# kongwanbianjinyu/PromptIR

Measured on AMD Instinct MI355X. Metric: 128x128 patches/sec (fwd+bwd train step, whole job), higher is better.
Workload: dtype f32 (bf16x3 split-MFMA, f32 accumulate)

## Files before the change

include/promptir_hip.h:

```cpp
#ifndef PROMPTIR_HIP_H
#define PROMPTIR_HIP_H

#include <stddef.h>
#include <stdint.h>

#ifdef __cplusplus
extern "C" {
#endif

#define PIR_OK 0
#define PIR_EINVAL (-22)
#define PIR_ENOMEM (-12)

typedef void* pir_stream_t;

int pir_abi_version(void);
const char* pir_arch(void);

int pir_tune_set(int knob, int value);

int pir_build_flags(void);

typedef struct {
  const float* A; long a_s1, a_s2; long a_sm, a_sk;
  const float* X; long x_s1, x_s2; long ldx;
  float* Y; long y_s1, y_s2; long ldy;
  const float* R; long r_s1, r_s2; long ldr;
  const float* rowscale; long rs_s1, rs_s2;
  int M, K, N;
  int O1, O2;
  const void* A3; int a3_kp;
} pir_gemm_nn_t;
int pir_gemm_nn(const pir_gemm_nn_t* args, pir_stream_t stream);
size_t pir_gemm_nn_ws_floats(const pir_gemm_nn_t* args);
int pir_gemm_nn_ws(const pir_gemm_nn_t* args, float* ws, size_t ws_floats, pir_stream_t stream);
int pir_ln_conv1x1_fwd(const float* x, long x_bs, const float* ln_w, const float* ln_b, const void* A3, int a3_kp,
                       float* y, long y_bs, float* mean_out, float* rstd_out, int B, int M, int K, int HW, pir_stream_t stream);
int pir_conv1x1_wgrad_ln(const float* dy, long dy_bs, const float* x, long x_bs, const float* mean, const float* rstd,
                         const float* ln_w, const float* ln_b, float* dw, float* ws, size_t ws_floats,
                         int B, int Cout, int Cin, int HW, pir_stream_t stream);

int pir_conv1x1_dgrad_ln_bwd(const float* dy, long dy_bs, const void* A3, int a3_kp, int K,
                             const float* x, long x_bs, const float* ln_w, const float* mean, const float* rstd,
                             const float* dres, long dres_bs, float* dx, long dx_bs, float* dweight, float* dbias,
                             float* ws, size_t ws_floats, int B, int C, int HW, pir_stream_t stream);

int pir_gemm_nn_plan(const pir_gemm_nn_t* args);
size_t pir_split_bf16x3_bytes(int M, int K);
int pir_split_bf16x3(const float* W, int M, int K, long sm, long sk, void* out, pir_stream_t stream);

int pir_conv3x3(const float* A, long a_st, long a_sm, long a_sk, int flip,
                const float* X, long x_bs, float* Y, long y_bs,
                const float* R, long r_bs,
                int B, int M, int K, int H, int W, pir_stream_t stream);

typedef struct {
  const float* X; long x_s1, x_s2, x_sr; long ldx;
  const float* Y; long y_s1, y_s2, y_sr; long ldy;
  float* G; long g_so, g_si, g_sj;
  int M1, M2, N;
  int O1, O2, BR;
  int shift_dh, shift_dw, H, W;
  float* ws; size_t ws_floats;
  float alpha;
  int accumulate;
} pir_gemm_nt_t;
size_t pir_gemm_nt_ws_floats(int M1, int M2, int N, int O, int BR);
int pir_gemm_nt(const pir_gemm_nt_t* args, pir_stream_t stream);
int pir_gemm_nt_partials(const pir_gemm_nt_t* args, int* splits, pir_stream_t stream);
int pir_gemm_nt_group(const pir_gemm_nt_t* probs, int n, pir_stream_t stream);
size_t pir_gemm_nt_ws_needed(const pir_gemm_nt_t* args);
size_t pir_gemm_nt_group_ws_needed(const pir_gemm_nt_t* probs, int n, int k);

int pir_split_bf16x3_taps(const float* W, int M, int K, long st, long sm, long sk, int flip, void* out,
                          pir_stream_t stream);
int pir_conv3x3_x3(const void* A3, int a3_kp, const float* X, long x_bs, float* Y, long y_bs,
                   const float* R, long r_bs, int B, int M, int K, int H, int W, pir_stream_t stream);
size_t pir_conv3x3_x3_ws_floats(int B, int M, int K, int H, int W);
int pir_conv3x3_x3_ws(const void* A3, int a3_kp, const float* X, long x_bs, float* Y, long y_bs,
                      const float* R, long r_bs, int B, int M, int K, int H, int W,
                      float* ws, size_t ws_floats, pir_stream_t stream);

typedef struct {
  const float* W; void* out;
  long st, sm, sk;
  int M, K, taps, flip;
} pir_split_desc_t;
int pir_split_bf16x3_batch(const pir_split_desc_t* descs, const int* blocks, int nblocks, pir_stream_t stream);

size_t pir_conv3x3_wgrad_ws_floats(int Cout, int Cin, int H, int W, int B);
int pir_conv3x3_wgrad(const float* dy, long dy_bs, const float* x, long x_bs, float* dw, int B, int Cout, int Cin,
                      int H, int W, float* ws, size_t ws_floats, int accumulate, pir_stream_t stream);

int pir_layernorm_fwd(const float* x, long x_bs, const float* weight, const float* bias,
                      float* y, long y_bs, float* mean, float* rstd,
                      int B, int C, int HW, pir_stream_t stream);
size_t pir_layernorm_bwd_ws_floats(int B, int C, int HW);
int pir_layernorm_bwd(const float* dy, long dy_bs, const float* x, long x_bs, const float* weight,
                      int with_bias, const float* mean, const float* rstd,
                      float* dx, long dx_bs, const float* dres, long dres_bs, float* dweight, float* dbias,
                      float* ws, size_t ws_floats, int B, int C, int HW, pir_stream_t stream);

int pir_dwconv3x3(const float* x, long x_bs, const float* w, int flip, float* y, long y_bs,
                  int B, int C, int H, int W, pir_stream_t stream);
size_t pir_dwconv3x3_sumsq_floats(int B, int nsq, int H);
int pir_dwconv3x3_sumsq(const float* x, long x_bs, const float* w, float* y, long y_bs, float* sq_parts,
                        size_t sq_floats, int nsq, int* nparts, int B, int C, int H, int W, pir_stream_t stream);
int pir_dwconv3x3_gate(const float* x, long x_bs, const float* w, float* g, long g_bs,
                       int B, int hid, int H, int W, pir_stream_t stream);
int pir_dwconv3x3_gate_bwd(const float* x, long x_bs, const float* w, const float* dg, long dg_bs,
                           float* dt, long dt_bs, int B, int hid, int H, int W, pir_stream_t stream);
size_t pir_dwconv3x3_wgrad_ws_floats(int B, int C, int H, int W);
int pir_dwconv3x3_wgrad(const float* dy, long dy_bs, const float* x, long x_bs, float* dw,
                        float* ws, size_t ws_floats, int B, int C, int H, int W, pir_stream_t stream);

size_t pir_dwconv3x3_bwd_ws_floats(int B, int C, int H, int W);
int pir_dwconv3x3_bwd(const float* dy, long dy_bs, const float* x, long x_bs, const float* w,
                      float* dx, long dx_bs, float* dw, float* ws, size_t ws_floats,
                      int B, int C, int H, int W, pir_stream_t stream);
size_t pir_gdfn_dwconv_bwd_ws_floats(int B, int hid, int H, int W);
int pir_gdfn_dwconv_bwd(const float* x, long x_bs, const float* w, const float* dg, long dg_bs,
                        float* dx, long dx_bs, float* dw, float* ws, size_t ws_floats,
                        int B, int hid, int H, int W, pir_stream_t stream);

int pir_row_sumsq(const float* x, long x_bs, float* out, int B, int C, int HW, pir_stream_t stream);
int pir_mdta_softmax_fwd(const float* gram, const float* sumsq, int nparts, const float* temperature,
                         float* attn, int B, int heads, int c, pir_stream_t stream);
int pir_mdta_softmax_fwd_parts(const float* gram_parts, int splits, const float* sumsq, int nparts,
                               const float* temperature, float* gram, float* attn, int B, int heads, int c,
                               pir_stream_t stream);
// ... 77 lines not shown
```

promptir_amd/_lib.py:

```python
from __future__ import annotations

import ctypes as C
import os

_HERE = os.path.dirname(os.path.abspath(__file__))
LIB_PATH = os.environ.get("PIR_LIB", os.path.join(_HERE, "libpromptir_hip.so"))
ABI_VERSION = 8

c_float_p = C.c_void_p
c_long = C.c_long
c_int = C.c_int
c_size_t = C.c_size_t
c_float = C.c_float
stream_t = C.c_void_p


class GemmNN(C.Structure):
    _fields_ = [
        ("A", c_float_p), ("a_s1", c_long), ("a_s2", c_long), ("a_sm", c_long), ("a_sk", c_long),
        ("X", c_float_p), ("x_s1", c_long), ("x_s2", c_long), ("ldx", c_long),
        ("Y", c_float_p), ("y_s1", c_long), ("y_s2", c_long), ("ldy", c_long),
        ("R", c_float_p), ("r_s1", c_long), ("r_s2", c_long), ("ldr", c_long),
        ("rowscale", c_float_p), ("rs_s1", c_long), ("rs_s2", c_long),
        ("M", c_int), ("K", c_int), ("N", c_int), ("O1", c_int), ("O2", c_int),
        ("A3", c_float_p), ("a3_kp", c_int),
    ]


class GemmNT(C.Structure):
    _fields_ = [
        ("X", c_float_p), ("x_s1", c_long), ("x_s2", c_long), ("x_sr", c_long), ("ldx", c_long),
        ("Y", c_float_p), ("y_s1", c_long), ("y_s2", c_long), ("y_sr", c_long), ("ldy", c_long),
        ("G", c_float_p), ("g_so", c_long), ("g_si", c_long), ("g_sj", c_long),
        ("M1", c_int), ("M2", c_int), ("N", c_int), ("O1", c_int), ("O2", c_int), ("BR", c_int),
        ("shift_dh", c_int), ("shift_dw", c_int), ("H", c_int), ("W", c_int),
        ("ws", c_float_p), ("ws_floats", c_size_t),
        ("alpha", c_float), ("accumulate", c_int),
    ]


class SplitDesc(C.Structure):
    _fields_ = [("W", c_float_p), ("out", c_float_p), ("st", c_long), ("sm", c_long), ("sk", c_long),
                ("M", c_int), ("K", c_int), ("taps", c_int), ("flip", c_int)]


P, L, I, Z, F, S = c_float_p, c_long, c_int, c_size_t, c_float, stream_t

SIGNATURES = {
    "pir_abi_version": (I, []),
    "pir_arch": (C.c_char_p, []),
    "pir_tune_set": (I, [I, I]),
    "pir_build_flags": (I, []),
    "pir_gemm_nn": (I, [C.POINTER(GemmNN), S]),
    "pir_gemm_nn_ws": (I, [C.POINTER(GemmNN), P, Z, S]),
    "pir_gemm_nn_ws_floats": (Z, [C.POINTER(GemmNN)]),
    "pir_gemm_nn_plan": (I, [C.POINTER(GemmNN)]),
    "pir_split_bf16x3_bytes": (Z, [I, I]),
    "pir_split_bf16x3": (I, [P, I, I, L, L, P, S]),
    "pir_conv3x3": (I, [P, L, L, L, I, P, L, P, L, P, L, I, I, I, I, I, S]),
    "pir_gemm_nt_ws_floats": (Z, [I, I, I, I, I]),
    "pir_gemm_nt": (I, [C.POINTER(GemmNT), S]),
    "pir_gemm_nt_partials": (I, [C.POINTER(GemmNT), C.POINTER(C.c_int), S]),
    "pir_gemm_nt_group": (I, [C.POINTER(GemmNT), I, S]),
    "pir_gemm_nt_ws_needed": (Z, [C.POINTER(GemmNT)]),
    "pir_gemm_nt_group_ws_needed": (Z, [C.POINTER(GemmNT), I, I]),
    "pir_split_bf16x3_batch": (I, [P, P, I, S]),
    "pir_split_bf16x3_taps": (I, [P, I, I, L, L, L, I, P, S]),
    "pir_conv3x3_x3": (I, [P, I, P, L, P, L, P, L, I, I, I, I, I, S]),
    "pir_conv3x3_x3_ws": (I, [P, I, P, L, P, L, P, L, I, I, I, I, I, P, Z, S]),
    "pir_conv3x3_x3_ws_floats": (Z, [I, I, I, I, I]),
    "pir_conv3x3_wgrad_ws_floats": (Z, [I, I, I, I, I]),
    "pir_conv3x3_wgrad": (I, [P, L, P, L, P, I, I, I, I, I, P, Z, I, S]),
    "pir_layernorm_fwd": (I, [P, L, P, P, P, L, P, P, I, I, I, S]),
    "pir_layernorm_bwd_ws_floats": (Z, [I, I, I]),
    "pir_layernorm_bwd": (I, [P, L, P, L, P, I, P, P, P, L, P, L, P, P, P, Z, I, I, I, S]),
    "pir_dwconv3x3": (I, [P, L, P, I, P, L, I, I, I, I, S]),
    "pir_dwconv3x3_gate": (I, [P, L, P, P, L, I, I, I, I, S]),
    "pir_dwconv3x3_gate_bwd": (I, [P, L, P, P, L, P, L, I, I, I, I, S]),
    "pir_dwconv3x3_wgrad_ws_floats": (Z, [I, I, I, I]),
    "pir_dwconv3x3_wgrad": (I, [P, L, P, L, P, P, Z, I, I, I, I, S]),
    "pir_dwconv3x3_bwd_ws_floats": (Z, [I, I, I, I]),
    "pir_dwconv3x3_bwd": (I, [P, L, P, L, P, P, L, P, P, Z, I, I, I, I, S]),
    "pir_gdfn_dwconv_bwd_ws_floats": (Z, [I, I, I, I]),
    "pir_gdfn_dwconv_bwd": (I, [P, L, P, P, L, P, L, P, P, Z, I, I, I, I, S]),
    "pir_gdfn_fused_ws_bytes": (Z, [I, I, I, I]),
    "pir_gdfn_fused_fwd": (I, [P, L, P, P, P, I, P, P, L, P, Z, P, P, I, I, I, I, I, S]),
    "pir_row_sumsq": (I, [P, L, P, I, I, I, S]),
    "pir_mdta_softmax_fwd": (I, [P, P, I, P, P, I, I, I, S]),
    "pir_mdta_softmax_bwd": (I, [P, P, P, P, I, P, P, P, P, P, I, I, I, S]),
    "pir_mdta_softmax_fwd_parts": (I, [P, I, P, I, P, P, P, I, I, I, S]),
    "pir_mdta_softmax_bwd_parts": (I, [P, I, P, P, P, I, P, P, P, P, P, I, I, I, S]),
    "pir_dwconv3x3_sumsq_floats": (Z, [I, I, I]),
    "pir_dwconv3x3_sumsq": (I, [P, L, P, P, L, P, Z, I, C.POINTER(C.c_int), I, I, I, I, S]),
    "pir_pixel_unshuffle2": (I, [P, L, P, L, I, I, I, I, S]),
    "pir_pixel_shuffle2": (I, [P, L, P, L, I, I, I, I, S]),
    "pir_spatial_mean": (I, [P, L, P, I, I, I, S]),
    "pir_prompt_mix_fwd": (I, [P, P, P, P, I, I, I, S]),
    "pir_prompt_resize_fwd": (I, [P, P, P, L, I, I, I, I, I, I, S]),
    "pir_prompt_resize_bwd_ws_floats": (Z, [I, I, I, I, I, I]),
    "pir_prompt_resize_bwd": (I, [P, L, P, P, P, P, P, Z, I, I, I, I, I, I, S]),
    "pir_prompt_mix_bwd": (I, [P, P, P, P, P, P, P, L, I, I, I, I, I, S]),
    "pir_tiles_gather": (I, [P, L, P, I, I, I, I, I, I, I, I, I, I, I, I, I, S]),
    "pir_tiles_blend": (I, [P, P, L, I, I, I, I, I, I, I, I, I, I, I, I, I, S]),
    "pir_l1_loss": (I, [P, P, P, P, F, F, P, L, S]),
    "pir_l1_loss_grad": (I, [P, P, P, F, P, L, S]),
    "pir_copy_strided4": (I, [P, L, L, L, L, P, I, I, I, I, S]),
    "pir_degrade_gaussian": (I, [P, P, P, P, L, I, S]),
    "pir_crop_augment_u8": (I, [P, P, P, P, P, P, I, I, S]),
    "pir_copy_planes": (I, [P, L, P, L, I, I, L, S]),
    "pir_add": (I, [P, P, P, L, S]),
    "pir_bias_add": (I, [P, L, P, I, I, I, S]),
    "pir_bias_grad": (I, [P, L, P, I, I, I, S]),
    "pir_gelu_gate": (I, [P, L, P, L, I, I, I, S]),
    "pir_gelu_gate_bwd": (I, [P, L, P, L, P, L, I, I, I, S]),
    "pir_reduce_partials": (I, [P, L, I, F, I, P, L, S]),
    "pir_reduce_defer": (I, [S, I]),
    "pir_reduce_flush": (I, [S]),
    "pir_reduce_pending": (I, [S]),
    "pir_reduce_defer_limit": (L, [L]),
    "pir_ln_conv1x1_fwd": (I, [P, L, P, P, P, I, P, L, P, P, I, I, I, I, S]),
    "pir_conv1x1_wgrad_ln": (I, [P, L, P, L, P, P, P, P, P, P, Z, I, I, I, I, S]),
    "pir_conv1x1_dgrad_ln_bwd": (I, [P, L, P, I, I, P, L, P, P, P, P, L, P, L, P, P, P, Z, I, I, I, S]),
    "pir_mdta_dqk": (I, [P, P, L, L, P, P, P, L, L, I, I, I, I, S]),
    "pir_adamw_step": (I, [P, P, P, P, L, F, F, F, F, F, L, F, S]),
}


class HipLibraryError(RuntimeError):
    pass


def _load() -> C.CDLL:
    if not os.path.exists(LIB_PATH):
        raise HipLibraryError(
            f"{LIB_PATH} not found: build it with `python -c 'import __graft_entry__ as g; g.build()'` "
            "(or `make -C promptir_amd/csrc`). promptir_amd has no CPU / eager fallback.")
    lib = C.CDLL(LIB_PATH)
    for name, (restype, argtypes) in SIGNATURES.items():
        try:
# ... 29 lines not shown
```

promptir_amd/csrc/gemm.hip:

```cpp
#include "gemm_common.h"
#include <stdlib.h>


namespace {

#ifndef PIR_BK
#define PIR_BK 16
#endif
constexpr int BK = PIR_BK;
#ifndef PIR_PIN_SCHED
#define PIR_PIN_SCHED 0
#endif
constexpr bool PIN_SCHED = PIR_PIN_SCHED;

int g_nn_cfg = -1, g_nt_cfg = -1, g_nt_splits = 0, g_nn_x3 = -1, g_nt_x3 = -1;
int g_nt_want_half = 5;
int g_nt_group_wide = 0;
int g_nt_tile96 = 0;
int g_nt_quad = -1;

__device__ __forceinline__ int c_row(int reg, int lane) { return pir_c_row(reg, lane); }

struct NNParams {
  pir_gemm_nn_t g;
// ... 778 lines not shown
  };
  const bool vec4 = (g.H == 0 || tap_sign != 0) && g.N % 4 == 0 && al(g.X, g.x_s1, g.x_s2, g.x_sr, g.ldx) &&
                    al(g.Y, g.y_s1, g.y_s2, g.y_sr, g.ldy);
  const bool x3 = vec4 && (g_nt_x3 != 0 || tap_sign != 0);
  if (tap_sign != 0 && !x3) return PIR_EINVAL;
  if ((long)g.BR * pir_cdiv(g.N, x3 ? X3_BK : NT_BK) >= 2147483647L) return PIR_EINVAL;
  NTPlan pl = nt_plan(g.M1, g.M2, g.N, O, g.BR, x3 ? X3_BK : NT_BK, x3 && tap_sign == 0, tap_sign != 0);
  int xp_splits = 0;
  if (x3 && tap_sign == 0 && g_nt_cfg < 0 && g_nt_splits == 0) {
    const int st = pir_nt_xp_launch(&g, &xp_splits, s);
    if (st != 1000 && st != PIR_OK) return st;
    if (st == 1000) xp_splits = 0;
  }
  if (xp_splits > 0) pl.splits = xp_splits;
  if ((size_t)pl.splits * O * g.M1 * g.M2 > ws_floats) return PIR_ENOMEM;
  p.splits = pl.splits;
  p.chunks_per_r = pl.chunks_per_r;
  p.tap_sign = tap_sign;
  p.magic_w = pir_magic(g.W > 0 ? (unsigned)g.W : 1u);
  dim3 grid((unsigned)(pir_cdiv(g.M1, pl.bm) * pir_cdiv(g.M2, pl.bn)), (unsigned)pl.splits, (unsigned)O);
  if (xp_splits > 0) {
  } else if (tap_sign != 0) {
    switch (pl.cfg) {
      case 0: hipLaunchKernelGGL((gemm_nt_x3_kernel<1, 1, 2, 2, true>), grid, dim3(256), 0, s, p); break;
      case 1: hipLaunchKernelGGL((gemm_nt_x3_kernel<2, 1, 2, 2, true>), grid, dim3(256), 0, s, p); break;
      case 2: hipLaunchKernelGGL((gemm_nt_x3_kernel<1, 3, 4, 1, true>), grid, dim3(256), 0, s, p); break;
      case 6: hipLaunchKernelGGL((gemm_nt_x3_kernel<1, 2, 2, 2, true>), grid, dim3(256), 0, s, p); break;
      default: hipLaunchKernelGGL((gemm_nt_x3_kernel<2, 2, 2, 2, true>), grid, dim3(256), 0, s, p); break;
    }
  } else if (x3 && (g_nt_quad < 0 ? (g.N >= 1024 && pl.cfg != 1) : g_nt_quad != 0)) {
    switch (pl.cfg) {
      case 0: hipLaunchKernelGGL((gemm_nt_x3_kernel<1, 1, 2, 2, false, true>), grid, dim3(256), 0, s, p); break;
      case 1: hipLaunchKernelGGL((gemm_nt_x3_kernel<2, 1, 2, 2, false, true>), grid, dim3(256), 0, s, p); break;
      case 2: hipLaunchKernelGGL((gemm_nt_x3_kernel<1, 3, 4, 1, false, true>), grid, dim3(256), 0, s, p); break;
      case 4: hipLaunchKernelGGL((gemm_nt_x3_kernel<1, 3, 8, 1, false, true>), grid, dim3(512), 0, s, p); break;
      case 5: hipLaunchKernelGGL((gemm_nt_x3_kernel<2, 2, 4, 2, false, true>), grid, dim3(512), 0, s, p); break;
      case 7: hipLaunchKernelGGL((gemm_nt_x3_kernel<1, 3, 3, 1, false, true>), grid, dim3(192), 0, s, p); break;
      default: hipLaunchKernelGGL((gemm_nt_x3_kernel<2, 2, 2, 2, false, true>), grid, dim3(256), 0, s, p); break;
    }
  } else if (x3) {
    switch (pl.cfg) {
      case 0: hipLaunchKernelGGL((gemm_nt_x3_kernel<1, 1, 2, 2>), grid, dim3(256), 0, s, p); break;
      case 1: hipLaunchKernelGGL((gemm_nt_x3_kernel<2, 1, 2, 2>), grid, dim3(256), 0, s, p); break;
      case 2: hipLaunchKernelGGL((gemm_nt_x3_kernel<1, 3, 4, 1>), grid, dim3(256), 0, s, p); break;
      case 4: hipLaunchKernelGGL((gemm_nt_x3_kernel<1, 3, 8, 1>), grid, dim3(512), 0, s, p); break;
      case 5: hipLaunchKernelGGL((gemm_nt_x3_kernel<2, 2, 4, 2>), grid, dim3(512), 0, s, p); break;
      case 7: hipLaunchKernelGGL((gemm_nt_x3_kernel<1, 3, 3, 1>), grid, dim3(192), 0, s, p); break;
      default: hipLaunchKernelGGL((gemm_nt_x3_kernel<2, 2, 2, 2>), grid, dim3(256), 0, s, p); break;
    }
  } else {
    switch (pl.cfg) {
      case 0: launch_nt_cfg<2, 2, 1, 1, 4>(p, grid, vec4, s); break;
      case 1: launch_nt_cfg<2, 2, 2, 1, 2>(p, grid, vec4, s); break;
      case 2: launch_nt_cfg<2, 3, 2, 1, 2>(p, grid, vec4, s); break;
      default: launch_nt_cfg<2, 2, 2, 2, 1>(p, grid, vec4, s); break;
    }
  }
  int st = pir_launch_status();
  if (st) return st;
  if (partials_only) { *partials_only = pl.splits; return PIR_OK; }
  return pir_nt_reduce_submit(g.ws, pl.splits, O, g.M1, g.M2, g.G, g.g_so, g.g_si, g.g_sj, g_st, g.alpha, g.accumulate, s);
}

}

int pir_nt_reduce_launch(const float* ws, int splits, int M1, int M2, float* G, long g_so, long g_si, long g_sj, float alpha,
                         int accumulate, hipStream_t s) {
  return pir_nt_reduce_submit(ws, splits, 1, M1, M2, G, g_so, g_si, g_sj, 0L, alpha, accumulate, s);
}

int pir_gdfn_wave_tune(int knob, int value);
int pir_stencil_wave_tune(int knob, int value);
int pir_ln_tune(int knob, int value);
int pir_gdfn_fused_tune(int knob, int value);
int pir_mdta_dqk_tune(int knob, int value);

extern "C" int pir_tune_set(int knob, int value) {
  switch (knob) {
    case 0: g_nn_cfg = value; return PIR_OK;
    case 1: g_nt_cfg = value; return PIR_OK;
    case 2: g_nt_splits = value; return PIR_OK;
    case 3: g_nn_x3 = value; return PIR_OK;
    case 4: g_nt_x3 = value; return PIR_OK;
    case 5: case 18: case 29: case 43: case 44: case 45: return pir_nn_x3_tune(knob, value);
    case 6: case 7: return pir_gdfn_wave_tune(knob, value);
    case 8: case 9: case 10: return pir_stencil_wave_tune(knob, value);
    case 13: case 16: return pir_ln_tune(knob, value);
    case 14: g_nt_quad = value; return PIR_OK;
    case 33: g_nt_tile96 = value; return PIR_OK;
    case 34: g_nt_group_wide = value; return PIR_OK;
    case 35: case 37: return pir_gdfn_fused_tune(knob, value);
    case 36: return pir_mdta_dqk_tune(knob, value);
    case 19: g_nt_want_half = value; return PIR_OK;
    case 20: return pir_nn_res_tune(knob, value);
    case 21: case 22: case 23: case 24: return pir_nn_res_tune2(knob, value);
    case 25: case 38: case 40: return pir_nt_xp_tune(knob, value);
    case 26: case 27: case 32: return pir_nn_cst_tune(knob, value);
    case 30: return pir_conv_rows_tune(knob, value);
    default: return PIR_EINVAL;
  }
}

extern "C" int pir_gemm_nn_plan(const pir_gemm_nn_t* a) {
  if (!a || a->M <= 0 || a->K <= 0 || a->N <= 0 || a->O1 <= 0 || a->O2 <= 0) return PIR_EINVAL;
  if (!pir_nn_x3_wanted(a, g_nn_x3)) return 0;
  if (g_nn_cfg < 0) {
    if (pir_nn_cst_serves(a)) return 9200;
    const int kind = pir_nn_res_kind(a);
    if (kind) return kind == 2 ? 9100 : 9000;
  }
  return pir_nn_x3_plan(a, g_nn_cfg);
}

int pir_reduce_partials_now(const float* parts, long stride, int S, float alpha, int accumulate, float* out, long count,
                            pir_stream_t stream);

static int nn_x3_tiled(const pir_gemm_nn_t* a) {
  if (!pir_nn_x3_wanted(a, g_nn_x3)) return 0;
  if (g_nn_cfg < 0 && (pir_nn_cst_serves(a) || pir_nn_res_kind(a))) return 0;
  return 1;
}

extern "C" size_t pir_gemm_nn_ws_floats(const pir_gemm_nn_t* a) {
  if (!a || a->M <= 0 || a->K <= 0 || a->N <= 0 || a->O1 <= 0 || a->O2 <= 0 || !nn_x3_tiled(a)) return 0;
  const int sp = pir_nn_x3_ksplit(a, g_nn_cfg);
  return sp > 1 ? (size_t)sp * a->O1 * a->M * a->N : 0;
}

static int gemm_nn_impl(const pir_gemm_nn_t* a, float* ws, size_t ws_floats, pir_stream_t stream) {
  PIR_CHECK_ARG(a && a->A && a->X && a->Y);
  PIR_CHECK_ARG(a->M > 0 && a->K > 0 && a->N > 0 && a->O1 > 0 && a->O2 > 0);
  PIR_CHECK_ARG((long)a->O1 * a->O2 <= 65535);
  PIR_CHECK_ARG(a->rowscale == nullptr || a->R != nullptr);
  PIR_CHECK_ARG((long)a->M * a->ldy < 2147483647L && (long)a->K * a->ldx < 2147483647L);
  PIR_CHECK_ARG(a->R == nullptr || (long)a->M * a->ldr < 2147483647L);
  PIR_CHECK_ARG((long)(a->M - 1) * a->a_sm + (long)(a->K - 1) * a->a_sk < 2147483647L);
  if (pir_nn_x3_wanted(a, g_nn_x3)) {
    if (g_nn_cfg < 0) {
      int st = pir_nn_cst_launch(a, (hipStream_t)stream);
      if (st != 1000) return st;
      st = pir_nn_res_launch(a, (hipStream_t)stream);
      if (st != 1000) return st;
    }
    const int sp = ws ? pir_nn_x3_ksplit(a, g_nn_cfg) : 1;
    const long out_floats = (long)a->O1 * a->M * a->N;
    if (sp > 1 && (size_t)sp * out_floats <= ws_floats && (reinterpret_cast<uintptr_t>(ws) & 15) == 0) {
      pir_gemm_nn_t gs = *a;
      gs.Y = ws;
      const int st = pir_nn_x3_launch(&gs, g_nn_cfg, (hipStream_t)stream, sp, out_floats);
      if (st) return st;
      return pir_reduce_partials_now(ws, out_floats, sp, 1.f, 0, a->Y, out_floats, stream);
    }
    return pir_nn_x3_launch(a, g_nn_cfg, (hipStream_t)stream);
  }
  NNParams p;
  p.g = *a;
  p.taps = 1; p.flip = 0; p.H = 0; p.W = 0; p.a_st = 0;
  return launch_nn(p, (hipStream_t)stream);
}

extern "C" int pir_gemm_nn(const pir_gemm_nn_t* a, pir_stream_t stream) { return gemm_nn_impl(a, nullptr, 0, stream); }

extern "C" int pir_gemm_nn_ws(const pir_gemm_nn_t* a, float* ws, size_t ws_floats, pir_stream_t stream) {
  return gemm_nn_impl(a, ws, ws_floats, stream);
}

extern "C" int pir_conv3x3(const float* A, long a_st, long a_sm, long a_sk, int flip,
                           const float* X, long x_bs, float* Y, long y_bs,
                           const float* R, long r_bs,
                           int B, int M, int K, int H, int W, pir_stream_t stream) {
  PIR_CHECK_ARG(A && X && Y && B > 0 && M > 0 && K > 0 && H > 0 && W > 0 && B <= 65535);
  PIR_CHECK_ARG((long)(M > K ? M : K) * H * W < 2147483647L);
  NNParams p;
  pir_gemm_nn_t& g = p.g;
  g.A = A; g.a_s1 = 0; g.a_s2 = 0; g.a_sm = a_sm; g.a_sk = a_sk;
  g.X = X; g.x_s1 = x_bs; g.x_s2 = 0; g.ldx = (long)H * W;
  g.Y = Y; g.y_s1 = y_bs; g.y_s2 = 0; g.ldy = (long)H * W;
  g.R = R; g.r_s1 = r_bs; g.r_s2 = 0; g.ldr = (long)H * W;
  g.rowscale = nullptr; g.rs_s1 = 0; g.rs_s2 = 0;
  g.M = M; g.K = K; g.N = H * W; g.O1 = B; g.O2 = 1; g.A3 = nullptr; g.a3_kp = 0;
  p.taps = 9; p.flip = flip; p.H = H; p.W = W; p.a_st = a_st;
  return launch_nn(p, (hipStream_t)stream);
}

extern "C" size_t pir_gemm_nt_ws_floats(int M1, int M2, int N, int O, int BR) {
  if (M1 <= 0 || M2 <= 0 || N <= 0 || O <= 0 || BR <= 0) return 0;
  NTPlan a = nt_plan(M1, M2, N, O, BR), b = nt_plan(M2, M1, N, O, BR);
  NTPlan c = nt_plan(M1, M2, N, O, BR, X3_BK), d = nt_plan(M2, M1, N, O, BR, X3_BK);
  NTPlan e = nt_plan(M1, M2, N, O, BR, X3_BK, true), f = nt_plan(M2, M1, N, O, BR, X3_BK, true);
  int s = a.splits > b.splits ? a.splits : b.splits;
  if (c.splits > s) s = c.splits;
  if (d.splits > s) s = d.splits;
  if (e.splits > s) s = e.splits;
  if (f.splits > s) s = f.splits;
// ... 196 lines not shown
```

promptir_amd/csrc/gemm_common.h:

```cpp
#pragma once
#include "pir_common.h"

__device__ __forceinline__ int pir_c_row(int reg, int lane) { return (reg & 3) + 8 * (reg >> 2) + 4 * (lane >> 5); }

template <int TM, int TN>
__device__ __forceinline__ void pir_nn_epilogue(const f32x16 (&acc)[TM][TN], const pir_gemm_nn_t& g, float* __restrict__ Y,
                                                int o1, int o2, int m0, int n0, int wm, int wn, int lane) {
  const float* __restrict__ R = g.R ? g.R + o1 * g.r_s1 + o2 * g.r_s2 : nullptr;
  const float* __restrict__ RS = g.rowscale ? g.rowscale + o1 * g.rs_s1 + o2 * g.rs_s2 : nullptr;
  const int ldy = (int)g.ldy, ldr = (int)g.ldr;
#pragma unroll
  for (int i = 0; i < TM; ++i)
#pragma unroll
    for (int j = 0; j < TN; ++j) {
      const int nb = n0 + (wn * TN + j) * 32, mb = m0 + (wm * TM + i) * 32;
      const int n = nb + (lane & 31), mrow = mb + 4 * (lane >> 5);
      const bool full = mb + 32 <= g.M && nb + 32 <= g.N;
      if (full) {
        const int offy = mrow * ldy + n;
        float res[16];
        if (R) {
          const int offr = mrow * ldr + n;
#pragma unroll
          for (int r = 0; r < 16; ++r) res[r] = R[offr + ((r & 3) + 8 * (r >> 2)) * ldr];
          if (RS) {
#pragma unroll
            for (int r = 0; r < 16; ++r) res[r] *= RS[mrow + (r & 3) + 8 * (r >> 2)];
          }
#pragma unroll
          for (int r = 0; r < 16; ++r) Y[offy + ((r & 3) + 8 * (r >> 2)) * ldy] = acc[i][j][r] + res[r];
        } else {
#pragma unroll
          for (int r = 0; r < 16; ++r) Y[offy + ((r & 3) + 8 * (r >> 2)) * ldy] = acc[i][j][r];
        }
      } else {
        const int nc = n < g.N ? n : g.N - 1;
        float res[16];
        if (R) {
#pragma unroll
          for (int r = 0; r < 16; ++r) {
            const int m = mrow + (r & 3) + 8 * (r >> 2);
            const int mc = m < g.M ? m : g.M - 1;
            res[r] = R[mc * ldr + nc] * (RS ? RS[mc] : 1.f);
          }
        }
#pragma unroll
        for (int r = 0; r < 16; ++r) {
          const int m = mrow + (r & 3) + 8 * (r >> 2);
          if (m < g.M && n < g.N) Y[m * ldy + n] = R ? acc[i][j][r] + res[r] : acc[i][j][r];
        }
      }
    }
}

typedef __bf16 pir_bf16x8 __attribute__((ext_vector_type(8)));
struct pir_frag3 { pir_bf16x8 hi, mid, lo; };

__device__ __forceinline__ pir_frag3 pir_split8(const float (&v)[8]) {
  pir_frag3 f;
#pragma unroll
  for (int j = 0; j < 8; ++j) {
    const float x = v[j];
    const __bf16 h = (__bf16)x;
    const float r1 = x - (float)h;
    const __bf16 m = (__bf16)r1;
    const float r2 = r1 - (float)m;
    f.hi[j] = h; f.mid[j] = m; f.lo[j] = (__bf16)r2;
  }
  return f;
}

typedef __bf16 pir_bf16x4 __attribute__((ext_vector_type(4)));
struct pir_frag3h { pir_bf16x4 hi, mid, lo; };
__device__ __forceinline__ pir_frag3h pir_split4(const float (&v)[4]) {
  pir_frag3h f;
#pragma unroll
  for (int j = 0; j < 4; ++j) {
    const float x = v[j];
    const __bf16 h = (__bf16)x;
    const float r1 = x - (float)h;
    const __bf16 m = (__bf16)r1;
    const float r2 = r1 - (float)m;
    f.hi[j] = h; f.mid[j] = m; f.lo[j] = (__bf16)r2;
  }
  return f;
}

__device__ __forceinline__ f32x16 pir_mfma_x3(const pir_bf16x8& ah, const pir_bf16x8& am, const pir_bf16x8& al,
                                              const pir_bf16x8& bh, const pir_bf16x8& bm, const pir_bf16x8& bl, f32x16 c) {
  c = __builtin_amdgcn_mfma_f32_32x32x16_bf16(al, bh, c, 0, 0, 0);
  c = __builtin_amdgcn_mfma_f32_32x32x16_bf16(ah, bl, c, 0, 0, 0);
  c = __builtin_amdgcn_mfma_f32_32x32x16_bf16(am, bm, c, 0, 0, 0);
  c = __builtin_amdgcn_mfma_f32_32x32x16_bf16(am, bh, c, 0, 0, 0);
  c = __builtin_amdgcn_mfma_f32_32x32x16_bf16(ah, bm, c, 0, 0, 0);
  c = __builtin_amdgcn_mfma_f32_32x32x16_bf16(ah, bh, c, 0, 0, 0);
  return c;
}

bool pir_nn_x3_wanted(const pir_gemm_nn_t* a, int knob);
int pir_nn_x3_launch(const pir_gemm_nn_t* a, int cfg, hipStream_t stream, int ksplit = 1, long part_stride = 0);
int pir_nn_x3_ksplit(const pir_gemm_nn_t* a, int cfg);
int pir_nn_x3_plan(const pir_gemm_nn_t* a, int cfg);
int pir_nn_x3_tune(int knob, int value);

int pir_nn_res_kind(const pir_gemm_nn_t* a);
int pir_nn_res_launch(const pir_gemm_nn_t* a, hipStream_t stream);
int pir_nn_res_tune(int knob, int value);
int pir_nn_res_tune2(int knob, int value);

int pir_conv_rows_launch(const pir_gemm_nn_t* g, int H, int W, int tile, hipStream_t stream, int splits = 1, long part_stride = 0);
bool pir_conv_rows_serves(const pir_gemm_nn_t* g, int W, int tile);
int pir_conv_rows_tune(int knob, int value);

bool pir_nn_cst_serves(const pir_gemm_nn_t* a);
int pir_nn_cst_launch(const pir_gemm_nn_t* a, hipStream_t stream);
int pir_nn_cst_tune(int knob, int value);

int pir_nt_xp_launch(const pir_gemm_nt_t* a, int* splits, hipStream_t stream, const float* y_mean = nullptr, const float* y_rstd = nullptr,
                     const float* y_gamma = nullptr, const float* y_beta = nullptr);
int pir_nt_xp_splits(const pir_gemm_nt_t* a);
int pir_nt_xp_tune(int knob, int value);
```

promptir_amd/csrc/gemm_x3.hip:

```cpp
#include "gemm_common.h"

namespace {

typedef __bf16 bf16x8 __attribute__((ext_vector_type(8)));
typedef unsigned int u32x4 __attribute__((ext_vector_type(4)));
constexpr int XK = 16;

struct Frag3 { bf16x8 hi, mid, lo; };

__device__ __forceinline__ Frag3 split8(const float (&v)[8], bool ok) {
  Frag3 f;
#pragma unroll
  for (int j = 0; j < 8; ++j) {
    const float x = ok ? v[j] : 0.f;
    const __bf16 h = (__bf16)x;
    const float r1 = x - (float)h;
    const __bf16 m = (__bf16)r1;
    const float r2 = r1 - (float)m;
    f.hi[j] = h; f.mid[j] = m; f.lo[j] = (__bf16)r2;
  }
  return f;
}

struct X3Conv { int H, W, ksteps; unsigned magic_ks, magic_w; int ksplit; long part_stride; };
// ... 139 lines not shown
    for (int q = 0; q < TM * TN * 6; ++q) {
      __builtin_amdgcn_sched_group_barrier(0x008, 1, 0);
      __builtin_amdgcn_sched_group_barrier(0x020, 1, 0);
    }
    __builtin_amdgcn_sched_group_barrier(0x200, 3 * NB, 0);
  };

  f32x16 acc[TM][TN];
#pragma unroll
  for (int i = 0; i < TM; ++i)
#pragma unroll
    for (int j = 0; j < TN; ++j)
#pragma unroll
      for (int r = 0; r < 16; ++r) acc[i][j][r] = 0.f;

  auto compute = [&](int buf) {
    const bf16x8* base = smem + buf * STAGE;
    const int h = lane >> 5, r = lane & 31;
    const bf16x8* ap = base + h * AKS + wm * TM * 32 + r;
    const bf16x8* bp = base + AU + h * BN + wn * TN * 32 + r;
    bf16x8 ah[TM], am[TM], al[TM], bh[TN], bm[TN], bl[TN];
#pragma unroll
    for (int i = 0; i < TM; ++i) { ah[i] = ap[i * 32]; am[i] = ap[PART + i * 32]; al[i] = ap[2 * PART + i * 32]; }
#pragma unroll
    for (int j = 0; j < TN; ++j) {
      if constexpr (BREG) { bh[j] = bfr[buf].hi; bm[j] = bfr[buf].mid; bl[j] = bfr[buf].lo; }
      else { bh[j] = bp[j * 32]; bm[j] = bp[PART + j * 32]; bl[j] = bp[2 * PART + j * 32]; }
    }
#define PIR_X3_TERM(A_, B_)                                                                   \
    _Pragma("unroll") for (int i = 0; i < TM; ++i) _Pragma("unroll") for (int j = 0; j < TN; ++j) \
        acc[i][j] = __builtin_amdgcn_mfma_f32_32x32x16_bf16(A_[i], B_[j], acc[i][j], 0, 0, 0);
    PIR_X3_TERM(al, bh)
    PIR_X3_TERM(ah, bl)
    PIR_X3_TERM(am, bm)
    PIR_X3_TERM(am, bh)
    PIR_X3_TERM(ah, bm)
    PIR_X3_TERM(ah, bh)
#undef PIR_X3_TERM
  };

  Stage s0, s1;
  load(0, s0);
  if (iters > 1) load(1, s1);
  stash(0, 0, s0);
  __syncthreads();
  int it = 0;
  for (; it + 3 < iters; it += 2) {
    load(it + 2, s0);
    compute(0);
    stash_b(1, s1);
    interleave();
    stash_a(1, it + 1, s1);
    __syncthreads();
    load(it + 3, s1);
    compute(1);
    stash_b(0, s0);
    interleave();
    stash_a(0, it + 2, s0);
    __syncthreads();
  }
  for (; it + 1 < iters; it += 2) {
    if (it + 2 < iters) load(it + 2, s0);
    compute(0);
    stash_b(1, s1);
    stash_a(1, it + 1, s1);
    __syncthreads();
    if (it + 3 < iters) load(it + 3, s1);
    compute(1);
    stash_b(0, s0);
    if (it + 2 < iters) stash_a(0, it + 2, s0);
    __syncthreads();
  }
  if (it < iters) compute(0);

  if (!CONV && blockIdx.z != 0) {
    pir_gemm_nn_t gz = g;
    gz.R = nullptr; gz.rowscale = nullptr;
    pir_nn_epilogue<TM, TN>(acc, gz, Y, o1, o2, m0, n0, wm, wn, lane);
    return;
  }
  pir_nn_epilogue<TM, TN>(acc, g, Y, o1, o2, m0, n0, wm, wn, lane);
}

int g_x3_fill32 = 45;
int g_x3_breg = -1;

int g_x3_conv_fill = 1;

template <int TM, int TN, int WM, int WN>
int launch_cfg(const pir_gemm_nn_t& g, hipStream_t s, const X3Conv* conv = nullptr, int ksplit = 1, long part_stride = 0) {
  constexpr int BM = WM * TM * 32, BN = WN * TN * 32;
  const long tiles = pir_cdiv(g.M, BM) * pir_cdiv(g.N, BN);
  dim3 grid((unsigned)tiles, (unsigned)(g.O1 * g.O2), (unsigned)(conv ? 1 : ksplit)), block(WM * WN * 64);
  X3Conv cv = {0, 0, 0, 0u, 0u, ksplit, part_stride};
  if (conv) hipLaunchKernelGGL((gemm_nn_x3_kernel<TM, TN, WM, WN, true, true, true>), grid, block, 0, s, g, *conv);
  else if (g.A3 && (g_x3_breg < 0 ? g.N <= 4096 : g_x3_breg != 0) && WM == 1 && TN == 1) {
    if constexpr (WM == 1 && TN == 1) hipLaunchKernelGGL((gemm_nn_x3_kernel<TM, TN, WM, WN, true, true, false, true>), grid, block, 0, s, g, cv);
  }
  else if (g.A3) hipLaunchKernelGGL((gemm_nn_x3_kernel<TM, TN, WM, WN, true, true>), grid, block, 0, s, g, cv);
  else if (g.a_sm == 1) hipLaunchKernelGGL((gemm_nn_x3_kernel<TM, TN, WM, WN, true, false>), grid, block, 0, s, g, cv);
  else hipLaunchKernelGGL((gemm_nn_x3_kernel<TM, TN, WM, WN, false, false>), grid, block, 0, s, g, cv);
  return pir_launch_status();
}

__global__ __launch_bounds__(256) void split_bf16x3_kernel(const float* __restrict__ W, int M, int K, long sm, long sk,
                                                           __bf16* __restrict__ out, int kp) {
  const long total = (long)M * kp;
  for (long e = blockIdx.x * (long)blockDim.x + threadIdx.x; e < total; e += (long)gridDim.x * blockDim.x) {
    const int m = (int)(e / kp), k = (int)(e % kp);
    const float x = k < K ? W[m * sm + k * sk] : 0.f;
    const __bf16 h = (__bf16)x;
    const float r1 = x - (float)h;
    const __bf16 mid = (__bf16)r1;
    const float r2 = r1 - (float)mid;
    const long d = ((long)(k >> 4) * M + m) * 16 + (k & 15);
    out[d] = h; out[total + d] = mid; out[2 * total + d] = (__bf16)r2;
  }
}

__global__ __launch_bounds__(256) void split_bf16x3_taps_kernel(const float* __restrict__ W, int M, int K, long st, long sm,
                                                                long sk, int flip, __bf16* __restrict__ out, int kp) {
  const long per_tap = (long)M * kp, total = 9 * per_tap;
  for (long e = blockIdx.x * (long)blockDim.x + threadIdx.x; e < total; e += (long)gridDim.x * blockDim.x) {
    const int tap = (int)(e / per_tap);
    const long r = e - tap * per_tap;
    const int m = (int)(r / kp), k = (int)(r % kp);
    const float x = k < K ? W[(flip ? 8 - tap : tap) * st + m * sm + k * sk] : 0.f;
    const __bf16 h = (__bf16)x;
    const float r1 = x - (float)h;
    const __bf16 mid = (__bf16)r1;
    const float r2 = r1 - (float)mid;
    const long d = tap * per_tap + ((long)(k >> 4) * M + m) * 16 + (k & 15);
    out[d] = h; out[total + d] = mid; out[2 * total + d] = (__bf16)r2;
  }
}

__global__ __launch_bounds__(256) void split_bf16x3_batch_kernel(const pir_split_desc_t* __restrict__ descs,
                                                                 const int2* __restrict__ blk) {
  const int2 bd = blk[blockIdx.x];
  const pir_split_desc_t d = descs[bd.x];
  const int kp = (d.K + 15) / 16 * 16, ntap = d.taps ? 9 : 1;
  const long per_tap = (long)d.M * kp, total = ntap * per_tap;
  const long per_step = (long)d.M * 16;
  __bf16* __restrict__ out = reinterpret_cast<__bf16*>(d.out);
  const long base = (long)bd.y * 4096;
#pragma unroll 4
  for (int i = 0; i < 16; ++i) {
    const long o = base + i * 256 + threadIdx.x;
    if (o >= total) break;
    const int tap = (int)(o / per_tap);
    const long r = o - tap * per_tap;
    const int ks = (int)(r / per_step);
    const int r2 = (int)(r - ks * per_step);
    const int m = r2 >> 4, k = ks * 16 + (r2 & 15);
    const float x = k < d.K ? d.W[(d.flip ? 8 - tap : tap) * d.st + m * d.sm + k * d.sk] : 0.f;
    const __bf16 h = (__bf16)x;
    const float r1 = x - (float)h;
    const __bf16 mid = (__bf16)r1;
    const float rr = r1 - (float)mid;
    out[o] = h; out[total + o] = mid; out[2 * total + o] = (__bf16)rr;
  }
}

}

extern "C" int pir_split_bf16x3_batch(const pir_split_desc_t* descs, const int* blocks, int nblocks, pir_stream_t stream) {
  PIR_CHECK_ARG(descs && blocks && nblocks > 0);
  hipLaunchKernelGGL(split_bf16x3_batch_kernel, dim3(nblocks), dim3(256), 0, (hipStream_t)stream, descs,
                     reinterpret_cast<const int2*>(blocks));
  return pir_launch_status();
}

extern "C" int pir_split_bf16x3_taps(const float* W, int M, int K, long st, long sm, long sk, int flip, void* out,
                                     pir_stream_t stream) {
  PIR_CHECK_ARG(W && out && M > 0 && K > 0 && (reinterpret_cast<uintptr_t>(out) & 15) == 0);
  const int kp = (int)(pir_cdiv(K, 16) * 16);
  const long total = 9L * M * kp;
  const int blocks = (int)(pir_cdiv(total, 256) < 2048 ? pir_cdiv(total, 256) : 2048);
  hipLaunchKernelGGL(split_bf16x3_taps_kernel, dim3(blocks), dim3(256), 0, (hipStream_t)stream, W, M, K, st, sm, sk, flip,
                     reinterpret_cast<__bf16*>(out), kp);
// ... 36 lines not shown
}

int pir_reduce_partials_now(const float* parts, long stride, int S, float alpha, int accumulate, float* out, long count,
                            pir_stream_t stream);

static int conv3x3_x3_impl(const void* A3, int a3_kp, const float* X, long x_bs, float* Y, long y_bs, const float* R,
                           long r_bs, int B, int M, int K, int H, int W, float* ws, size_t ws_floats, pir_stream_t stream) {
  PIR_CHECK_ARG(A3 && X && Y && B > 0 && M > 0 && K > 0 && H > 0 && W > 0 && B <= 65535);
  PIR_CHECK_ARG(a3_kp == (int)(pir_cdiv(K, 16) * 16));
  PIR_CHECK_ARG((long)(M > K ? M : K) * H * W < (1L << 28) && 54L * M * a3_kp < (1L << 31));
  PIR_CHECK_ARG(((long)H * W + 256) * W < (1L << 32));
  pir_gemm_nn_t g;
  g.A = nullptr; g.a_s1 = g.a_s2 = 0; g.a_sm = 0; g.a_sk = 0;
  g.X = X; g.x_s1 = x_bs; g.x_s2 = 0; g.ldx = (long)H * W;
  g.Y = Y; g.y_s1 = y_bs; g.y_s2 = 0; g.ldy = (long)H * W;
  g.R = R; g.r_s1 = r_bs; g.r_s2 = 0; g.ldr = (long)H * W;
  g.rowscale = nullptr; g.rs_s1 = g.rs_s2 = 0;
  g.M = M; g.K = K; g.N = H * W; g.O1 = B; g.O2 = 1;
  g.A3 = A3; g.a3_kp = a3_kp;
  X3Conv cv;
  cv.ksplit = 1; cv.part_stride = 0;
  cv.H = H; cv.W = W; cv.ksteps = a3_kp / 16;
  cv.magic_ks = pir_magic((unsigned)cv.ksteps); cv.magic_w = pir_magic((unsigned)W);
  hipStream_t s = (hipStream_t)stream;
  const int tile = conv_tile(M, g.N, B);
  const int sp = conv_splits(tile, M, g.N, B, a3_kp);
  const long out_floats = (long)B * M * g.N;
  if (sp > 1 && ws && (size_t)sp * out_floats <= ws_floats && y_bs == (long)M * g.N && (reinterpret_cast<uintptr_t>(ws) & 15) == 0 &&
      pir_conv_rows_serves(&g, W, tile)) {
    pir_gemm_nn_t gs = g;
    gs.Y = ws; gs.y_s1 = (long)M * g.N;
    int st = pir_conv_rows_launch(&gs, H, W, tile, s, sp, out_floats);
    if (st) return st;
    return pir_reduce_partials_now(ws, out_floats, sp, 1.f, 0, Y, out_floats, stream);
  }
  {
    const int st = pir_conv_rows_launch(&g, H, W, tile, s);
    if (st != 1000) return st;
  }
  switch (tile) {
    case 1214: return launch_cfg<1, 2, 1, 4>(g, s, &cv);
    case 2214: return launch_cfg<2, 2, 1, 4>(g, s, &cv);
    case 3214: return launch_cfg<3, 2, 1, 4>(g, s, &cv);
    case 3114: return launch_cfg<3, 1, 1, 4>(g, s, &cv);
    case 1222: return launch_cfg<1, 2, 2, 2>(g, s, &cv);
    default: return launch_cfg<2, 2, 2, 2>(g, s, &cv);
  }
}

extern "C" int pir_conv3x3_x3(const void* A3, int a3_kp, const float* X, long x_bs, float* Y, long y_bs, const float* R,
                              long r_bs, int B, int M, int K, int H, int W, pir_stream_t stream) {
  return conv3x3_x3_impl(A3, a3_kp, X, x_bs, Y, y_bs, R, r_bs, B, M, K, H, W, nullptr, 0, stream);
}

extern "C" int pir_conv3x3_x3_ws(const void* A3, int a3_kp, const float* X, long x_bs, float* Y, long y_bs, const float* R,
                                 long r_bs, int B, int M, int K, int H, int W, float* ws, size_t ws_floats, pir_stream_t stream) {
  return conv3x3_x3_impl(A3, a3_kp, X, x_bs, Y, y_bs, R, r_bs, B, M, K, H, W, ws, ws_floats, stream);
}

extern "C" size_t pir_split_bf16x3_bytes(int M, int K) {
  if (M <= 0 || K <= 0) return 0;
  return (size_t)3 * M * (pir_cdiv(K, 16) * 16) * 2;
}

extern "C" int pir_split_bf16x3(const float* W, int M, int K, long sm, long sk, void* out, pir_stream_t stream) {
  PIR_CHECK_ARG(W && out && M > 0 && K > 0 && (reinterpret_cast<uintptr_t>(out) & 15) == 0);
  const int kp = (int)(pir_cdiv(K, 16) * 16);
  const long total = (long)M * kp;
  const int blocks = (int)(pir_cdiv(total, 256) < 2048 ? pir_cdiv(total, 256) : 2048);
  hipLaunchKernelGGL(split_bf16x3_kernel, dim3(blocks), dim3(256), 0, (hipStream_t)stream, W, M, K, sm, sk,
                     reinterpret_cast<__bf16*>(out), kp);
  return pir_launch_status();
}

int g_x3_narrow96 = 4;

int pir_nn_x3_tune(int knob, int value) {
  if (knob == 5) { g_x3_narrow96 = value; return PIR_OK; }
  if (knob == 18) { g_x3_breg = value; return PIR_OK; }
  if (knob == 43) { g_x3_fill32 = value; return PIR_OK; }
  if (knob == 29) { g_x3_conv_fill = value; return PIR_OK; }
  if (knob == 44) { g_x3_conv_split = value; return PIR_OK; }
  if (knob == 45) { g_x3_ksplit = value; return PIR_OK; }
  return PIR_EINVAL;
}

bool pir_nn_x3_wanted(const pir_gemm_nn_t* a, int knob) {
  const long kp = pir_cdiv(a->K, 16) * 16;
  if ((kp * a->ldx + a->N) * 4 >= (1L << 31)) return false;
  return knob != 0;
}

int pir_nn_x3_plan(const pir_gemm_nn_t* a, int cfg) {
  const pir_gemm_nn_t& g = *a;
  const int M = g.M;
  const long batch = (long)g.O1 * g.O2;
  if (cfg >= 0) {
    switch (cfg) {
      case 0: return 1214;
      case 1: return 2214;
      case 2: return 3214;
      case 3: return 2222;
      case 7: return 3114;
      case 8: return 1114;
      default: return 1222;
    }
  }
  if (M <= 32) return 1214;
  if (M <= 64) return g.K <= 192 ? 1222 : 2214;
  const long pad96 = pir_cdiv(M, 96) * 96, pad128 = pir_cdiv(M, 128) * 128;
  if (g.A3 && g_x3_fill32 > 0 && M >= 64 && g.N <= 4096 &&
      pir_cdiv(M, 96) * pir_cdiv(g.N, 128) * batch * 100 < (long)g_x3_fill32 * PIR_NUM_CU) return 1114;
  if (g.A3 && M >= 192 && g.N <= 1024) return pad128 < pad96 ? 2222 : 3114;
  if (g.A3 && M >= 192 && g.N <= 4096 && g.K <= 128 && pad96 < pad128) return 3114;
  if (g.A3 && g.K <= 128 && g.N >= 4096 && M >= 192 && pad128 <= pad96) return 2222;
  if (g.A3 && g.K >= 384 && M == 96 && g.N >= 16384) return 3114;
  const bool use96 = g.N >= 1024 ? pad96 * 100 <= pad128 * 113 : pad96 < pad128;
  const long blocks = use96 ? pir_cdiv(M, 96) * pir_cdiv(g.N, 256) * batch : pir_cdiv(M, 128) * pir_cdiv(g.N, 128) * batch;
  if (blocks < 2L * PIR_NUM_CU && pir_cdiv(M, 64) * 64 <= pad128) return 1222;
  if (use96 && blocks < (long)g_x3_narrow96 * PIR_NUM_CU) return 3114;
  if (use96) return 3214;
  return 2222;
}


int pir_nn_x3_ksplit(const pir_gemm_nn_t* a, int cfg) {
  const pir_gemm_nn_t& g = *a;
  if (!g_x3_ksplit || !g.A3 || g.O2 != 1 || g.y_s1 != (long)g.M * g.N || g.ldy != g.N) return 1;
  const int plan = pir_nn_x3_plan(a, cfg);
  const int bm = (plan / 1000) * (plan / 10 % 10) * 32, bn = (plan / 100 % 10) * (plan % 10) * 32;
  const long wgs = pir_cdiv(g.M, bm) * pir_cdiv(g.N, bn) * g.O1;
  const int iters = (int)pir_cdiv(g.K, 16);
  if (wgs * 2 >= PIR_NUM_CU) return 1;
  long s = 2L * PIR_NUM_CU / wgs;
  if (s > iters / 16) s = iters / 16;
  if (s > 8) s = 8;
  return s < 2 ? 1 : (int)s;
}

int pir_nn_x3_launch(const pir_gemm_nn_t* a, int cfg, hipStream_t s, int ksplit, long part_stride) {
  const pir_gemm_nn_t& g = *a;
  switch (pir_nn_x3_plan(a, cfg)) {
    case 1214: return launch_cfg<1, 2, 1, 4>(g, s, nullptr, ksplit, part_stride);
    case 2214: return launch_cfg<2, 2, 1, 4>(g, s, nullptr, ksplit, part_stride);
    case 3214: return launch_cfg<3, 2, 1, 4>(g, s, nullptr, ksplit, part_stride);
    case 2222: return launch_cfg<2, 2, 2, 2>(g, s, nullptr, ksplit, part_stride);
    case 3114: return launch_cfg<3, 1, 1, 4>(g, s, nullptr, ksplit, part_stride);
    case 1114: return launch_cfg<1, 1, 1, 4>(g, s, nullptr, ksplit, part_stride);
    default: return launch_cfg<1, 2, 2, 2>(g, s, nullptr, ksplit, part_stride);
  }
}
```

Baseline: 352.7.

## Add 32-deep K staging kernel for B-register bf16x3 GEMM path

Adds a new GEMM kernel variant for the B-in-register, pre-split-A path that stages two 16-wide K steps per LDS stage (32 K per barrier). Next-stage global loads are interleaved with the 12 MFMA term groups under sched_barrier, and the kernel carries explicit waves-per-EU hints. It is selected by default when K exceeds 8 k-steps and the tile layout is TN=1, WM=1, WN=4. The intent is to halve the barrier count and hide load latency, at the cost of more registers and LDS per stage.

```diff
diff --git a/include/promptir_hip.h b/include/promptir_hip.h
--- a/include/promptir_hip.h
+++ b/include/promptir_hip.h
@@ -46,6 +46,7 @@
                              float* ws, size_t ws_floats, int B, int C, int HW, pir_stream_t stream);
 
 int pir_gemm_nn_plan(const pir_gemm_nn_t* args);
+int pir_gemm_nn_stage_depth(const pir_gemm_nn_t* args);
 size_t pir_split_bf16x3_bytes(int M, int K);
 int pir_split_bf16x3(const float* W, int M, int K, long sm, long sk, void* out, pir_stream_t stream);
 
diff --git a/promptir_amd/_lib.py b/promptir_amd/_lib.py
--- a/promptir_amd/_lib.py
+++ b/promptir_amd/_lib.py
@@ -55,6 +55,7 @@
     "pir_gemm_nn_ws": (I, [C.POINTER(GemmNN), P, Z, S]),
     "pir_gemm_nn_ws_floats": (Z, [C.POINTER(GemmNN)]),
     "pir_gemm_nn_plan": (I, [C.POINTER(GemmNN)]),
+    "pir_gemm_nn_stage_depth": (I, [C.POINTER(GemmNN)]),
     "pir_split_bf16x3_bytes": (Z, [I, I]),
     "pir_split_bf16x3": (I, [P, I, I, L, L, P, S]),
     "pir_conv3x3": (I, [P, L, L, L, I, P, L, P, L, P, L, I, I, I, I, I, S]),
diff --git a/promptir_amd/csrc/gemm.hip b/promptir_amd/csrc/gemm.hip
--- a/promptir_amd/csrc/gemm.hip
+++ b/promptir_amd/csrc/gemm.hip
@@ -884,7 +884,7 @@
     case 2: g_nt_splits = value; return PIR_OK;
     case 3: g_nn_x3 = value; return PIR_OK;
     case 4: g_nt_x3 = value; return PIR_OK;
-    case 5: case 18: case 29: case 43: case 44: case 45: return pir_nn_x3_tune(knob, value);
+    case 5: case 18: case 29: case 43: case 44: case 45: case 46: return pir_nn_x3_tune(knob, value);
     case 6: case 7: return pir_gdfn_wave_tune(knob, value);
     case 8: case 9: case 10: return pir_stencil_wave_tune(knob, value);
     case 13: case 16: return pir_ln_tune(knob, value);
@@ -912,6 +912,12 @@
     if (kind) return kind == 2 ? 9100 : 9000;
   }
   return pir_nn_x3_plan(a, g_nn_cfg);
+}
+
+extern "C" int pir_gemm_nn_stage_depth(const pir_gemm_nn_t* a) {
+  const int plan = pir_gemm_nn_plan(a);
+  if (plan < 0) return plan;
+  return plan == 0 || plan >= 9000 ? 0 : pir_nn_x3_stage_depth(a, plan);
 }
 
 int pir_reduce_partials_now(const float* parts, long stride, int S, float alpha, int accumulate, float* out, long count,
diff --git a/promptir_amd/csrc/gemm_common.h b/promptir_amd/csrc/gemm_common.h
--- a/promptir_amd/csrc/gemm_common.h
+++ b/promptir_amd/csrc/gemm_common.h
@@ -102,6 +102,7 @@
 int pir_nn_x3_ksplit(const pir_gemm_nn_t* a, int cfg);
 int pir_nn_x3_plan(const pir_gemm_nn_t* a, int cfg);
 int pir_nn_x3_tune(int knob, int value);
+int pir_nn_x3_stage_depth(const pir_gemm_nn_t* a, int plan);
 
 int pir_nn_res_kind(const pir_gemm_nn_t* a);
 int pir_nn_res_launch(const pir_gemm_nn_t* a, hipStream_t stream);
diff --git a/promptir_amd/csrc/gemm_x3.hip b/promptir_amd/csrc/gemm_x3.hip
--- a/promptir_amd/csrc/gemm_x3.hip
+++ b/promptir_amd/csrc/gemm_x3.hip
@@ -245,10 +245,142 @@
   pir_nn_epilogue<TM, TN>(acc, g, Y, o1, o2, m0, n0, wm, wn, lane);
 }
 
+template <int TM>
+__global__ __launch_bounds__(256) __attribute__((amdgpu_waves_per_eu(TM == 3 ? 3 : 2)))
+void gemm_nn_x3_breg32_kernel(pir_gemm_nn_t g, X3Conv cv) {
+  constexpr int BM = TM * 32, BN = 128, T = 256;
+  constexpr int AKS = BM + 4;
+  constexpr int AU = 2 * AKS, KSTEP = 3 * AU;
+  constexpr int STAGE = 2 * KSTEP;
+  __shared__ bf16x8 smem[2 * STAGE];
+
+  const int tid = threadIdx.x, lane = tid & 63, wn = tid >> 6;
+  const int tiles_m = (g.M + BM - 1) / BM;
+  const int wg = pir_xcd_remap(blockIdx.x, gridDim.x);
+  const int m0 = (wg % tiles_m) * BM, n0 = (wg / tiles_m) * BN;
+  const int o1 = blockIdx.y / g.O2, o2 = blockIdx.y % g.O2;
+  const float* __restrict__ X = g.X + o1 * g.x_s1 + o2 * g.x_s2;
+  float* __restrict__ Y = g.Y + o1 * g.y_s1 + o2 * g.y_s2 + (long)blockIdx.z * cv.part_stride;
+
+  const int iters_all = (g.K + XK - 1) / XK;
+  const int ks_per = cv.ksplit > 1 ? (iters_all + cv.ksplit - 1) / cv.ksplit : iters_all;
+  const int it_base = cv.ksplit > 1 ? (int)blockIdx.z * ks_per : 0;
+  const int iters = iters_all - it_base < ks_per ? iters_all - it_base : ks_per;
+  const int nst = (iters + 1) >> 1;
+
+  const __amdgpu_buffer_rsrc_t xrs = pir_make_rsrc(X, (unsigned)((((long)g.K - 1) * g.ldx + g.N) * 4));
+  const __amdgpu_buffer_rsrc_t ars = pir_make_rsrc(g.A3, (unsigned)(6L * g.M * g.a3_kp));
+  constexpr int AF = 2 * BM, NA = (2 * AF + T - 1) / T;
+  static_assert(AF % 64 == 0, "a wave's A fragments lie in one k-step");
+  int a_voff[NA], a_ks[NA], a_u[NA];
+#pragma unroll
+  for (int i = 0; i < NA; ++i) {
+    const int f = (tid + i * T) % (2 * AF), r = f % AF;
+    const int m = m0 + (r >> 1), mc = m < g.M ? m : g.M - 1;
+    a_voff[i] = (mc * 16 + 8 * (r & 1)) * 2;
+    a_ks[i] = __builtin_amdgcn_readfirstlane(f / AF);
+    a_u[i] = a_ks[i] * KSTEP + (r & 1) * AKS + (r >> 1);
+  }
+  const int b_voff = (n0 + wn * 32 + (lane & 31)) * 4 + (lane >> 5) * 8 * (int)g.ldx * 4;
+  const int a3_part_bytes = g.M * g.a3_kp * 2, a3_step_bytes = g.M * 32, ldx4 = (int)g.ldx * 4;
+
+  struct Stage { bf16x8 a3[NA][3]; float b[2][8]; };
+  constexpr int NLD = 3 * NA + 16;
+  auto load_one = [&](int s, int u, Stage& st) {
+    if (u < 3 * NA) {
+      const int i = u / 3, part = u % 3, kr = 2 * s + a_ks[i];
+      const int ks = it_base + (kr < iters ? kr : iters - 1);
+      st.a3[i][part] = __builtin_bit_cast(
+          bf16x8, __builtin_amdgcn_raw_buffer_load_b128(ars, a_voff[i], part * a3_part_bytes + ks * a3_step_bytes, 0));
+    } else if (u < NLD) {
+      const int j = (u - 3 * NA) / 8, q = (u - 3 * NA) % 8, kr = 2 * s + j;
+      const int k0 = (it_base + (kr < iters ? kr : iters - 1)) * XK;
+      st.b[j][q] = __builtin_bit_cast(float, __builtin_amdgcn_raw_buffer_load_b32(xrs, b_voff, (k0 + q) * ldx4, 0));
+    }
+  };
+  auto stash = [&](int buf, const Stage& st, Frag3 (&bfr)[2]) {
+    bf16x8* base = smem + buf * STAGE;
+#pragma unroll
+    for (int i = 0; i < NA; ++i) {
+      base[a_u[i]] = st.a3[i][0]; base[AU + a_u[i]] = st.a3[i][1]; base[2 * AU + a_u[i]] = st.a3[i][2];
+    }
+#pragma unroll
+    for (int j = 0; j < 2; ++j) bfr[j] = split8(st.b[j], true);
+  };
+
+  f32x16 acc[TM];
+#pragma unroll
+  for (int i = 0; i < TM; ++i)
+#pragma unroll
+    for (int r = 0; r < 16; ++r) acc[i][r] = 0.f;
+
+  struct AFrag { bf16x8 h[TM], m[TM], l[TM]; };
+  auto read_a = [&](int buf, int j, AFrag& a) {
+    const bf16x8* ap = smem + buf * STAGE + j * KSTEP + (lane >> 5) * AKS + (lane & 31);
+#pragma unroll
+    for (int i = 0; i < TM; ++i) { a.h[i] = ap[i * 32]; a.m[i] = ap[AU + i * 32]; a.l[i] = ap[2 * AU + i * 32]; }
+  };
+  auto term = [&](int t, const AFrag& a, const Frag3& b) {
+    const bf16x8* av = t == 0 ? a.l : (t == 1 || t == 4 || t == 5) ? a.h : a.m;
+    const bf16x8 bv = (t == 0 || t == 3 || t == 5) ? b.hi : t == 2 || t == 4 ? b.mid : b.lo;
+#pragma unroll
+    for (int i = 0; i < TM; ++i) acc[i] = __builtin_amdgcn_mfma_f32_32x32x16_bf16(av[i], bv, acc[i], 0, 0, 0);
+  };
+  auto kstep = [&](int buf, int j, const Frag3& b) {
+    AFrag a;
+    read_a(buf, j, a);
+#pragma unroll
+    for (int t = 0; t < 6; ++t) term(t, a, b);
+  };
+
+  Stage st;
+  Frag3 bcur[2];
+#pragma unroll
+  for (int u = 0; u < NLD; ++u) load_one(0, u, st);
+  stash(0, st, bcur);
+  __syncthreads();
+  int s = 0;
+  constexpr int LPT = (NLD + 11) / 12;
+  for (; s + 1 < nst; ++s) {
+    AFrag a0, a1;
+    read_a(s & 1, 0, a0);
+#pragma unroll
+    for (int t = 0; t < 12; ++t) {
+      if (t == 5) read_a(s & 1, 1, a1);
+      term(t % 6, t < 6 ? a0 : a1, bcur[t / 6]);
+#pragma unroll
+      for (int u = t * LPT; u < (t + 1) * LPT; ++u) load_one(s + 1, u, st);
+      __builtin_amdgcn_sched_barrier(0);
+    }
+    Frag3 bnext[2];
+    stash((s + 1) & 1, st, bnext);
+    __syncthreads();
+    bcur[0] = bnext[0]; bcur[1] = bnext[1];
+  }
+  kstep(s & 1, 0, bcur[0]);
+  if (2 * s + 1 < iters) kstep(s & 1, 1, bcur[1]);
+  f32x16 acc2[TM][1];
+#pragma unroll
+  for (int i = 0; i < TM; ++i) acc2[i][0] = acc[i];
+  if (blockIdx.z != 0) {
+    pir_gemm_nn_t gz = g;
+    gz.R = nullptr; gz.rowscale = nullptr;
+    pir_nn_epilogue<TM, 1>(acc2, gz, Y, o1, o2, m0, n0, 0, wn, lane);
+    return;
+  }
+  pir_nn_epilogue<TM, 1>(acc2, g, Y, o1, o2, m0, n0, 0, wn, lane);
+}
+
 int g_x3_fill32 = 45;
 int g_x3_breg = -1;
 
 int g_x3_conv_fill = 1;
+int g_x3_stage32 = -1;
+
+static bool x3_breg(const pir_gemm_nn_t& g) { return g.A3 && (g_x3_breg < 0 ? g.N <= 4096 : g_x3_breg != 0); }
+static bool x3_stage32(const pir_gemm_nn_t& g) {
+  return g_x3_stage32 < 0 ? g.K > 8 * XK : g_x3_stage32 != 0;
+}
 
 template <int TM, int TN, int WM, int WN>
 int launch_cfg(const pir_gemm_nn_t& g, hipStream_t s, const X3Conv* conv = nullptr, int ksplit = 1, long part_stride = 0) {
@@ -257,8 +389,11 @@
   dim3 grid((unsigned)tiles, (unsigned)(g.O1 * g.O2), (unsigned)(conv ? 1 : ksplit)), block(WM * WN * 64);
   X3Conv cv = {0, 0, 0, 0u, 0u, ksplit, part_stride};
   if (conv) hipLaunchKernelGGL((gemm_nn_x3_kernel<TM, TN, WM, WN, true, true, true>), grid, block, 0, s, g, *conv);
-  else if (g.A3 && (g_x3_breg < 0 ? g.N <= 4096 : g_x3_breg != 0) && WM == 1 && TN == 1) {
-    if constexpr (WM == 1 && TN == 1) hipLaunchKernelGGL((gemm_nn_x3_kernel<TM, TN, WM, WN, true, true, false, true>), grid, block, 0, s, g, cv);
+  else if (x3_breg(g) && WM == 1 && TN == 1) {
+    if constexpr (WM == 1 && TN == 1 && WN == 4) {
+      if (x3_stage32(g)) hipLaunchKernelGGL((gemm_nn_x3_breg32_kernel<TM>), grid, block, 0, s, g, cv);
+      else hipLaunchKernelGGL((gemm_nn_x3_kernel<TM, TN, WM, WN, true, true, false, true>), grid, block, 0, s, g, cv);
+    }
   }
   else if (g.A3) hipLaunchKernelGGL((gemm_nn_x3_kernel<TM, TN, WM, WN, true, true>), grid, block, 0, s, g, cv);
   else if (g.a_sm == 1) hipLaunchKernelGGL((gemm_nn_x3_kernel<TM, TN, WM, WN, true, false>), grid, block, 0, s, g, cv);
@@ -461,6 +596,7 @@
   if (knob == 29) { g_x3_conv_fill = value; return PIR_OK; }
   if (knob == 44) { g_x3_conv_split = value; return PIR_OK; }
   if (knob == 45) { g_x3_ksplit = value; return PIR_OK; }
+  if (knob == 46) { g_x3_stage32 = value; return PIR_OK; }
   return PIR_EINVAL;
 }
 
@@ -517,6 +653,11 @@
   return s < 2 ? 1 : (int)s;
 }
 
+int pir_nn_x3_stage_depth(const pir_gemm_nn_t* a, int plan) {
+  const int tm = plan / 1000, tn = plan / 100 % 10, wm = plan / 10 % 10, wn = plan % 10;
+  return tm && tn == 1 && wm == 1 && wn == 4 && x3_breg(*a) && x3_stage32(*a) ? 32 : 16;
+}
+
 int pir_nn_x3_launch(const pir_gemm_nn_t* a, int cfg, hipStream_t s, int ksplit, long part_stride) {
   const pir_gemm_nn_t& g = *a;
   switch (pir_nn_x3_plan(a, cfg)) {
```

Result: no change. 351.9, median of 6 (-0.2%).
